# schreibfaul1/ESP32-Opus-Player

Hardware: AMD Instinct MI355X
Metric: decoded 48 kHz stereo frames/sec/GPU (x real-time); HBM GB/s vs roofline (higher is better)
Workload: dtype int32 fixed-point (int16/int32 with 64-bit products); 1 GPU; celt_fb_stereo_64k; streams_per_gpu=65536

## Files before the change

### esp32-opus-player_amd/csrc/og_api.hip

```cpp
#include <hip/hip_runtime.h>
#include <stdio.h>
#include <stdlib.h>
#include <string.h>
#include <condition_variable>
#include <functional>
#include <memory>
#include <new>
#include <mutex>
#include <thread>
#include <vector>
#include "og_decode.hpp"
#include "og_host_framing.hpp"
#include "og_output.hpp"
#include "og_debug.hpp"

using namespace og;

static_assert(sizeof(opusgpu_frame_desc) == sizeof(FrameDesc), "descriptor layout");

#define OG_STALL_MAX_SPINS (1 << 20)
__global__ void __launch_bounds__(64) k_stream_stall(long long ticks, int max_spins) {
    const long long t0 = wall_clock64();
    for (int i = 0; i < max_spins && wall_clock64() - t0 < ticks; i++) __builtin_amdgcn_s_sleep(8);
}
// ... 148 lines not shown
        for (int k = 0; k < max_chunks; k++) consume(k, wa);
    }
    if (p < n) status[p] = st < 0 ? st : (i32)(crc == want);
}

static_assert(sizeof(opusgpu_output_cfg) == sizeof(OutputCfg) && sizeof(OutputCfg) == 4, "output cfg layout");
__global__ void __launch_bounds__(256) k_output_stage(const i16 *__restrict__ pcm, long long pcm_stride, const i32 *__restrict__ valid_of,
                                                       int valid_all, int block_samples, const OutputCfg *__restrict__ cfg_of,
                                                       OutputCfg cfg_all, u32 *__restrict__ out, long long out_stride,
                                                       int units_per_block, long long n_units, int vec_ok) {
    const long long t = (long long)blockIdx.x * 256 + threadIdx.x;
    if (t >= n_units) return;
    const int b = (int)(t / units_per_block), w0 = 4 * (int)(t - (long long)b * units_per_block);
    const OutputCfg c = cfg_of ? cfg_of[b] : cfg_all;
    int valid = valid_of ? valid_of[b] : valid_all;
    valid = valid > block_samples ? block_samples : valid;
    const int count = output_words(c, valid);
    if (w0 >= count) return;
    const i16 *blk = pcm + (size_t)b * pcm_stride;
    u32 *dst = out + (size_t)b * out_stride + w0;
    if (vec_ok && c.bits == 16 && c.channels == 2 && w0 + 4 <= count) {
        const uint4 v = *reinterpret_cast<const uint4 *>(blk + 2 * w0);
        const u32 in[4] = {v.x, v.y, v.z, v.w};
        u32 o[4];
#pragma unroll
        for (int j = 0; j < 4; j++) {
            i32 l = (i32)(i16)(in[j] & 0xffffu), r = (i32)(i16)(in[j] >> 16);
            if (c.force_mono) l = r = (i32)(i16)((l + r) / 2);
            o[j] = output_pack(l, r, false, (i32)c.volume);
        }
        *reinterpret_cast<uint4 *>(dst) = make_uint4(o[0], o[1], o[2], o[3]);
    } else {
        for (int j = 0; j < 4 && w0 + j < count; j++) dst[j] = output_word(blk, w0 + j, c);
    }
}

#ifndef OG_WAVES_PER_SIMD
#define OG_WAVES_PER_SIMD 1
#endif
#define OG_RECON_WAVES 2
#define OG_SILK_WAVES 2
__global__ void __launch_bounds__(64, OG_WAVES_PER_SIMD) k_decode_step(const FrameDesc *__restrict__ descs, const u8 *__restrict__ arena,
                                                   StreamState *st, i16 *pcm, i32 *result, int n, int n_streams,
                                                   int pcm_stride, int skip_celt, SilkHandoff *handoff, const SilkRec *srecs,
                                                   int q4_only) {
    unsigned long long todo = 1ull;
    int base = (int)blockIdx.x;
    if (q4_only) {
        base = (int)blockIdx.x * 64;
        const int f0 = base + (int)threadIdx.x;
        bool mine = false;
        if (f0 < n) {
            const FrameDesc d0 = descs[f0];
            mine = d0.stream >= 0 && d0.stream < n_streams && !desc_rfc(d0.flags) && desc_mode(d0.flags) == MODE_SILK && handoff[f0].valid == 2;
        }
        todo = __ballot(mine);
    }
    while (todo) {
        const int f = base + (int)__builtin_ctzll(todo);
        todo &= todo - 1;
        if (f >= n) return;
        const FrameDesc d = descs[f];
        int ret;
        if (d.stream < 0 || d.stream >= n_streams) {
            ret = BAD_ARG;
        } else if (desc_rfc(d.flags)) {
            continue;
        } else if (skip_celt && desc_mode(d.flags) == MODE_CELT) {
            continue;
        } else {
            StreamState *s = &st[d.stream];
#ifdef OG_PROF_SINGLE
            OG_PROF_INIT();
#endif
            ret = decode_frame_wave<true>(s, arena + d.offset, d.len, desc_mode(d.flags), desc_bandwidth(d.flags),
                                          desc_channels(d.flags), pcm + (size_t)f * pcm_stride, handoff ? &handoff[f] : nullptr,
                                          srecs ? &srecs[f] : nullptr, q4_only, desc_mode_after(d.flags));
#ifdef OG_PROF_SINGLE
            OG_PROF_FLUSH();
#endif
            if (ret == CONTINUE_SPLIT) continue;
        }
        if (threadIdx.x == 0) result[f] = ret;
        __syncthreads();
    }
}

extern "C" void og_launch_silk_synth(hipStream_t s, const void *descs, const void *arena, void *streams, void *pcm, void *result, int n,
                                     int n_streams, int pcm_stride, void *handoff, const void *srecs, int nb_elsewhere);
extern "C" void og_launch_silk_synth_nb(hipStream_t s, const void *descs, const void *arena, void *streams, void *pcm, void *result, int n,
                                        int n_streams, int pcm_stride, void *handoff, const void *srecs, int nb_elsewhere);

#define OG_SPARSE_WAVES 4
template <int LANES>
OG_DEV void silk_parse_kernel_body(const FrameDesc *__restrict__ descs, const u8 *__restrict__ arena, const StreamState *st, SilkRec *srecs,
                                   SilkHandoff *handoff, int n, int n_streams, SilkShadow *shadow, u32 epoch) {
    silk_tables_load();
    if ((int)threadIdx.x >= LANES) return;
    const int f = (int)blockIdx.x * LANES + (int)threadIdx.x;
    if (f >= n) return;
    const FrameDesc d = descs[f];
    const int mode = desc_mode(d.flags);
    if (d.stream < 0 || d.stream >= n_streams || mode == MODE_CELT || desc_rfc(d.flags)) return;
#ifdef OG_PROF_SPARSE
    OG_PROF_INIT();
#endif
    SilkShadow *const sh = shadow ? &shadow[d.stream] : nullptr;
    const SilkPast past(&st[d.stream], sh, epoch);
    silk_parse_lane(past, arena + d.offset, d.len, mode, desc_bandwidth(d.flags), desc_channels(d.flags), &srecs[f], &handoff[f], sh, epoch,
                    desc_mode_after(d.flags));
#ifdef OG_PROF_SPARSE
    OG_PROF_FLUSH();
#endif
}
__global__ void __launch_bounds__(64, OG_SPARSE_WAVES) k_silk_parse(const FrameDesc *__restrict__ descs, const u8 *__restrict__ arena,
                                                      const StreamState *st, SilkRec *srecs, SilkHandoff *handoff, int n,
                                                      int n_streams, SilkShadow *shadow, u32 epoch) {
    silk_parse_kernel_body<32>(descs, arena, st, srecs, handoff, n, n_streams, shadow, epoch);
}
__global__ void __launch_bounds__(64, OG_SPARSE_WAVES) k_silk_parse64(const FrameDesc *__restrict__ descs, const u8 *__restrict__ arena,
                                                        const StreamState *st, SilkRec *srecs, SilkHandoff *handoff, int n,
                                                        int n_streams, SilkShadow *shadow, u32 epoch) {
    silk_parse_kernel_body<64>(descs, arena, st, srecs, handoff, n, n_streams, shadow, epoch);
}

#define OG_SPARAMS_WAVES 4
__global__ void __launch_bounds__(64, OG_SPARAMS_WAVES) k_silk_params(const FrameDesc *__restrict__ descs, const StreamState *st, SilkRec *srecs,
                                                                       int n, int n_streams, SilkShadow *shadow, u32 epoch) {
    constexpr int FR = OG_PAR_LANES / 2;
    const int ch = (int)threadIdx.x / FR, f = (int)blockIdx.x * FR + (int)threadIdx.x % FR;
    bool act = f < n;
    FrameDesc d = {0, 0, 0, 0};
    if (act) {
        d = descs[f];
        act = !(d.stream < 0 || d.stream >= n_streams || desc_mode(d.flags) == MODE_CELT || desc_rfc(d.flags));
    }
    SilkShadow *const sh = act && shadow ? &shadow[d.stream] : nullptr;
    const SilkParPast past(act ? &st[d.stream] : st, sh, epoch);
    const int mode = desc_mode(d.flags), channels = desc_channels(d.flags);
    SilkParTask t;
    t.skip = 1;
    if (act) silk_params_channel(past, mode, desc_bandwidth(d.flags), channels, &srecs[f], ch, t);
    OG_FULL_SYNC();
    if (act) silk_params_shadow(past, t, channels, &srecs[f], ch, sh, epoch);
}

#define OG_PARSE_KERNEL_NAME k_celt_parse
#include "og_parse_kernel.hpp"
extern "C" void og_launch_celt_parse64(hipStream_t s, int grid, const void *descs, const void *arena, void *streams, void *recs, int n,
                                       int n_streams, const void *handoff, int which, int groups, unsigned *started);
extern "C" int og_celt_parse64_frames(void);

extern "C" void og_launch_celt_recon_fb(hipStream_t s, const void *descs, void *streams, const void *recs, void *rout, int n,
                                        int n_streams, int hybrid, unsigned *started);
extern "C" int og_celt_recon_fb_signals(int n);
extern "C" void og_launch_decode_rfc(hipStream_t s, const void *descs, const void *arena, void *streams, void *pcm, void *result, int n,
                                     int n_streams, int pcm_stride);
__global__ void __launch_bounds__(64, OG_RECON_WAVES) k_celt_recon(const FrameDesc *__restrict__ descs, StreamState *st,
                                                                      const ParseRec *recs, ReconOut *rout, int n,
                                                                      int n_streams, int hybrid, int rest_only) {
    unsigned long long todo = 1ull;
    int base = (int)blockIdx.x;
    if (rest_only) {
        base = (int)blockIdx.x * 64;
        const int f0 = base + (int)threadIdx.x;
        bool mine = false;
        if (f0 < n) {
            const FrameDesc d0 = descs[f0];
            const int m0 = desc_mode(d0.flags);
            if (d0.stream >= 0 && d0.stream < n_streams && (m0 == MODE_CELT || (m0 == MODE_HYBRID && hybrid)) && !desc_rfc(d0.flags)) {
                const u32 fl = recs[f0].flags;
                const bool fast = !(fl & (RF_SKIP | RF_BAD_CELT)) && ((fl >> RF_LM_SHIFT) & 3) == 3 && recs[f0].n_words < REC_MAX_WORDS &&
                                  recs[f0].n_leaves <= FAST_MAX_LEAVES;
                mine = !fast && !(m0 == MODE_HYBRID && (fl & RF_SKIP));
            }
        }
        todo = __ballot(mine);
    }
    while (todo) {
        const int f = base + (int)__builtin_ctzll(todo);
        todo &= todo - 1;
        if (f >= n) return;
        const FrameDesc d = descs[f];
        const int mode = desc_mode(d.flags);
        if (d.stream < 0 || d.stream >= n_streams || !(mode == MODE_CELT || (mode == MODE_HYBRID && hybrid)) || desc_rfc(d.flags)) continue;
        if (mode == MODE_HYBRID && (recs[f].flags & RF_SKIP)) continue;
#if !defined(OG_PROF_PARSE) && !defined(OG_PROF_SINGLE) && !defined(OG_PROF_SPARSE) && !defined(OG_PROF_SSYNTH)
        OG_PROF_INIT();
#endif
        const int pos = OG_UNI(st[d.stream].celt.ring_pos);
        const int ret = celt_recon_wave(&st[d.stream], &recs[f], mode, desc_channels(d.flags), rest_only ? RECON_REST_ONLY : RECON_ALL, desc_mode_after(d.flags));
        if (ret != RECON_NOT_MINE && threadIdx.x == 0) rout[f] = ReconOut{ret, pos};
#if !defined(OG_PROF_PARSE) && !defined(OG_PROF_SINGLE) && !defined(OG_PROF_SPARSE) && !defined(OG_PROF_SSYNTH)
        OG_PROF_FLUSH();
#endif
        __syncthreads();
    }
}

static __device__ __forceinline__ i32 pk_add_sat_i16(i32 a, i32 b) {
    typedef short s2 __attribute__((ext_vector_type(2)));
    const s2 r = __builtin_elementwise_add_sat(__builtin_bit_cast(s2, a), __builtin_bit_cast(s2, b));
    return __builtin_bit_cast(i32, r);
}
__global__ void __launch_bounds__(64) k_celt_post(const FrameDesc *__restrict__ descs, StreamState *st, const ParseRec *recs,
                                                  const ReconOut *__restrict__ rout, i32 *__restrict__ result, i16 *pcm, int n,
                                                  int n_streams, int channels, int pcm_stride, const SilkHandoff *handoff,
                                                  int modes, int others_ran) {
    struct RowInfo {
        const i32 *ring;
        i16 *pcm;
        const i16 *silk;
        int pos, silk_n;
    };
    constexpr int CS = 32, PCS = CS / 4, RSTEP = 64 / PCS;
    __shared__ RowInfo rows[64];
    __shared__ __attribute__((aligned(16))) i32 tin[64][CS + 4];
    __shared__ __attribute__((aligned(16))) i16 tout[64][CS + 8];
    const int lane = (int)threadIdx.x;
    const int t = (int)blockIdx.x * 64 + lane;
    const int f = channels == 2 ? t >> 1 : t, c = channels == 2 ? t & 1 : 0;
    bool live = false, emit = false;
    StreamState *ss = nullptr;
    const i16 *silk = nullptr;
    int silk_n = 0;
    int pos = 0;
    if (f < n) {
        const FrameDesc d = descs[f];
        const int mode = desc_mode(d.flags);
        const bool stream_ok = d.stream >= 0 && d.stream < n_streams;
        if (!(modes >> (d.flags & 3) & 1) || (!stream_ok && !others_ran)) {
            if (c == 0) result[f] = BAD_ARG;
        } else if (stream_ok && (mode == MODE_CELT || (mode == MODE_HYBRID && handoff)) && !desc_rfc(d.flags)) {
            const u32 rf = recs[f].flags;
            if (!(mode == MODE_HYBRID && (rf & RF_SKIP))) {
                const ReconOut ro = rout[f];
                if (c == 0) result[f] = ro.ret;
                if (!(rf & (RF_SKIP | RF_BAD_CELT))) {
                    live = true;
                    ss = &st[d.stream];
                    emit = ro.ret >= 0;
                    pos = ro.pos & RING_MASK;
                    if (mode == MODE_HYBRID) {
                        silk = handoff[f].pcm;
                        silk_n = 960 * desc_channels(d.flags);
                    }
                }
            }
        }
    }
    i16 *out = pcm + (size_t)(f < n ? f : 0) * pcm_stride;
    const bool fast = channels == 2 && __all(live && emit && (pos & (CS - 1)) == 0);
    if (!fast) {
        if (live) celt_post_lane(&ss->celt, c, channels, 960, pos, emit ? out : nullptr, silk, silk_n);
        return;
    }
    rows[lane].ring = ss->celt.ring[c];
    rows[lane].pcm = out;
    rows[lane].silk = silk;
    rows[lane].pos = pos;
    rows[lane].silk_n = silk_n;
    __syncthreads();
    const int q = lane % PCS, r0 = lane / PCS;
    const i32 *src[PCS];
    int spos[PCS];
#pragma unroll
    for (int k = 0; k < PCS; k++) {
        src[k] = rows[r0 + RSTEP * k].ring;
        spos[k] = rows[r0 + RSTEP * k].pos + 4 * q;
    }
    og_v4i v[PCS];
#pragma unroll
    for (int k = 0; k < PCS; k++) v[k] = *reinterpret_cast<const og_v4i *>(src[k] + (spos[k] & RING_MASK));
    i32 m = ss->celt.deemph[c];
    for (int ch = 0; ch < 960 / CS; ch++) {
#pragma unroll
        for (int k = 0; k < PCS; k++) *reinterpret_cast<og_v4i *>(&tin[r0 + RSTEP * k][4 * q]) = v[k];
        if (ch + 1 < 960 / CS) {
#pragma unroll
            for (int k = 0; k < PCS; k++) v[k] = *reinterpret_cast<const og_v4i *>(src[k] + ((spos[k] + CS * (ch + 1)) & RING_MASK));
        }
        __syncthreads();
#pragma unroll
        for (int g8 = 0; g8 < CS / 8; g8++) {
            i16 o[8];
#pragma unroll
            for (int h = 0; h < 2; h++) {
                const og_v4i sv = *reinterpret_cast<const og_v4i *>(&tin[lane][8 * g8 + 4 * h]);
                i32 tt = sv.x + m;
                m = mul16x32_q15(27853, tt);
                o[4 * h + 0] = (i16)sat16(pshr32(tt, 12));
                tt = sv.y + m;
                m = mul16x32_q15(27853, tt);
                o[4 * h + 1] = (i16)sat16(pshr32(tt, 12));
                tt = sv.z + m;
                m = mul16x32_q15(27853, tt);
                o[4 * h + 2] = (i16)sat16(pshr32(tt, 12));
                tt = sv.w + m;
                m = mul16x32_q15(27853, tt);
                o[4 * h + 3] = (i16)sat16(pshr32(tt, 12));
            }
            og_v4i w;
            w.x = (i32)((u32)(u16)o[0] | (u32)(u16)o[1] << 16);
            w.y = (i32)((u32)(u16)o[2] | (u32)(u16)o[3] << 16);
            w.z = (i32)((u32)(u16)o[4] | (u32)(u16)o[5] << 16);
            w.w = (i32)((u32)(u16)o[6] | (u32)(u16)o[7] << 16);
            *reinterpret_cast<og_v4i *>(&tout[lane][8 * g8]) = w;
        }
        __syncthreads();
#pragma unroll
        for (int k = 0; k < PCS / 2; k++) {
            const int fr = r0 + RSTEP * k;
            const og_v2u L = *reinterpret_cast<const og_v2u *>(&tout[2 * fr][4 * q]);
            const og_v2u R = *reinterpret_cast<const og_v2u *>(&tout[2 * fr + 1][4 * q]);
            og_v4i w;
            w.x = (i32)((L.x & 0xffffu) | R.x << 16);
            w.y = (i32)(L.x >> 16 | (R.x & 0xffff0000u));
            w.z = (i32)((L.y & 0xffffu) | R.y << 16);
            w.w = (i32)(L.y >> 16 | (R.y & 0xffff0000u));
            const int at = (CS * ch + 4 * q) * 2;
            const i16 *const sk = rows[2 * fr].silk;
            if (sk && at < rows[2 * fr].silk_n) {
                const og_v4i a = *reinterpret_cast<const og_v4i *>(sk + at);
                w.x = pk_add_sat_i16(w.x, a.x);
                w.y = pk_add_sat_i16(w.y, a.y);
                w.z = pk_add_sat_i16(w.z, a.z);
                w.w = pk_add_sat_i16(w.w, a.w);
            }
            *reinterpret_cast<og_v4i *>(rows[2 * fr].pcm + at) = w;
        }
    }
    ss->celt.deemph[c] = m;
}

#include "og_step.hpp"

const size_t og_parse_rec_bytes = sizeof(ParseRec), og_recon_out_bytes = sizeof(ReconOut), og_silk_handoff_bytes = sizeof(SilkHandoff),
             og_silk_rec_bytes = sizeof(SilkRec);
namespace {
struct StepRange {
    const FrameDesc *dd;
    i16 *pp;
    i32 *rr;
    ParseRec *recs;
    ReconOut *rout;
    SilkHandoff *hh;
    SilkRec *srecs;
    StepRange(const Step &st, size_t f0)
        : dd((const FrameDesc *)st.descs + f0), pp((i16 *)st.pcm + f0 * (size_t)st.pcm_stride), rr((i32 *)st.result + f0),
          recs((ParseRec *)st.recs + f0), rout((ReconOut *)st.rout + f0), hh(st.handoff ? (SilkHandoff *)st.handoff + f0 : nullptr),
          srecs(st.srecs ? (SilkRec *)st.srecs + f0 : nullptr) {}
};
}
void launch_stream_stall(opusgpu_ctx *ctx, hipStream_t q) {
    hipLaunchKernelGGL(k_stream_stall, dim3(1), dim3(64), 0, q, ctx->stall_ticks, (int)OG_STALL_MAX_SPINS);
}
void launch_decode_rfc(opusgpu_ctx *ctx, hipStream_t q, const Step &st) {
    og_launch_decode_rfc(q, st.descs, st.arena, ctx->d_streams, st.pcm, st.result, st.n, ctx->n_streams, st.pcm_stride);
}
void launch_decode_step(opusgpu_ctx *ctx, hipStream_t q, const Step &st, size_t f0, int cnt, int pass) {
    const StepRange r(st, f0);
    hipLaunchKernelGGL(k_decode_step, dim3(pass == 2 ? (cnt + 63) / 64 : cnt), dim3(64), 0, q, r.dd, (const u8 *)st.arena, ctx->d_streams, r.pp,
                       r.rr, cnt, ctx->n_streams, st.pcm_stride, pass ? 1 : 0, pass == 2 ? r.hh : nullptr,
                       (const SilkRec *)(pass == 2 ? r.srecs : nullptr), pass == 2 ? 1 : 0);
}
void launch_silk_parse(opusgpu_ctx *ctx, hipStream_t q, const Step &st, size_t f0, int cnt, void *shadow, uint32_t epoch) {
    const StepRange r(st, f0);
    hipLaunchKernelGGL(k_silk_parse, dim3((cnt + 31) / 32), dim3(64), 0, q, r.dd, (const u8 *)st.arena, (const StreamState *)ctx->d_streams,
                       r.srecs, r.hh, cnt, ctx->n_streams, (SilkShadow *)shadow, epoch);
}
void launch_silk_parse64(opusgpu_ctx *ctx, hipStream_t q, const Step &st, size_t f0, int cnt, void *shadow, uint32_t epoch) {
    const StepRange r(st, f0);
    hipLaunchKernelGGL(k_silk_parse64, dim3((cnt + 63) / 64), dim3(64), 0, q, r.dd, (const u8 *)st.arena, (const StreamState *)ctx->d_streams,
                       r.srecs, r.hh, cnt, ctx->n_streams, (SilkShadow *)shadow, epoch);
}
void launch_silk_params(opusgpu_ctx *ctx, hipStream_t q, const Step &st, size_t f0, int cnt, void *shadow, uint32_t epoch) {
    const StepRange r(st, f0);
    hipLaunchKernelGGL(k_silk_params, dim3((cnt + OG_PAR_LANES / 2 - 1) / (OG_PAR_LANES / 2)), dim3(64), 0, q, r.dd,
                       (const StreamState *)ctx->d_streams, r.srecs, cnt, ctx->n_streams, (SilkShadow *)shadow, epoch);
}
int celt_parse_early_grid(const opusgpu_ctx *ctx, int cnt, bool wide) {
    const int per = (wide ? og_celt_parse64_frames() : OG_PL_FRAMES) * ctx->parse_groups;
    return (cnt + per - 1) / per;
}
void launch_celt_parse(opusgpu_ctx *ctx, hipStream_t q, const Step &st, size_t f0, int cnt, bool wide, bool early) {
    const StepRange r(st, f0);
    const int which = early ? (int)PARSE_CELT_ONLY : (int)PARSE_ALL, groups = early ? ctx->parse_groups : 1;
    const int per = wide ? og_celt_parse64_frames() : OG_PL_FRAMES;
    const int grid = early ? celt_parse_early_grid(ctx, cnt, wide) : (cnt + per - 1) / per;
    u32 *const started = early ? ctx->sp.d_started : nullptr;
    if (wide)
        og_launch_celt_parse64(q, grid, r.dd, st.arena, ctx->d_streams, r.recs, cnt, ctx->n_streams, r.hh, which, groups, started);
    else
        hipLaunchKernelGGL(k_celt_parse, dim3(grid), dim3(64 * OG_PL_WAVES), 0, q, r.dd, (const u8 *)st.arena, ctx->d_streams, r.recs, cnt,
                           ctx->n_streams, (const SilkHandoff *)r.hh, which, groups, started);
}
void launch_celt_recon_fb(opusgpu_ctx *ctx, hipStream_t q, const Step &st, size_t f0, int cnt, bool counts_in) {
    const StepRange r(st, f0);
    og_launch_celt_recon_fb(q, r.dd, ctx->d_streams, r.recs, r.rout, cnt, ctx->n_streams, r.hh ? 1 : 0, counts_in ? ctx->sp.d_started + 16 : nullptr);
}
void launch_celt_recon(opusgpu_ctx *ctx, hipStream_t q, const Step &st, size_t f0, int cnt) {
    const StepRange r(st, f0);
    hipLaunchKernelGGL(k_celt_recon, dim3(ctx->fast_recon ? (cnt + 63) / 64 : cnt), dim3(64), 0, q, r.dd, ctx->d_streams, (const ParseRec *)r.recs,
                       r.rout, cnt, ctx->n_streams, r.hh ? 1 : 0, ctx->fast_recon);
}
void launch_celt_post(opusgpu_ctx *ctx, hipStream_t q, const Step &st, size_t f0, int cnt, bool others) {
    const StepRange r(st, f0);
    hipLaunchKernelGGL(k_celt_post, dim3((cnt * ctx->channels + 63) / 64), dim3(64), 0, q, r.dd, ctx->d_streams, (const ParseRec *)r.recs,
                       (const ReconOut *)r.rout, r.rr, r.pp, cnt, ctx->n_streams, ctx->channels, st.pcm_stride, (const SilkHandoff *)r.hh, st.modes,
                       others ? 1 : 0);
}
void launch_silk_synth(opusgpu_ctx *ctx, hipStream_t q, const Step &st, size_t f0, int cnt, int nb_done) {
    const StepRange r(st, f0);
    og_launch_silk_synth(q, r.dd, st.arena, ctx->d_streams, r.pp, r.rr, cnt, ctx->n_streams, st.pcm_stride, r.hh, r.srecs, nb_done);
}
void launch_silk_synth_nb(opusgpu_ctx *ctx, hipStream_t q, const Step &st, size_t f0, int cnt) {
    const StepRange r(st, f0);
    og_launch_silk_synth_nb(q, r.dd, st.arena, ctx->d_streams, r.pp, r.rr, cnt, ctx->n_streams, st.pcm_stride, r.hh, r.srecs, 1);
}


extern "C" {


int opusgpu_version(void) { return 100; }

int opusgpu_ctx_create(int device, opusgpu_ctx **out) {
    if (!out || device < 0) return OPUSGPU_BAD_ARG;
    *out = nullptr;
    int count = 0;
    if (hipGetDeviceCount(&count) != hipSuccess || count <= 0 || device >= count) return OPUSGPU_ERR_NO_DEVICE;
    if (hipSetDevice(device) != hipSuccess) return OPUSGPU_ERR_NO_DEVICE;
    hipFuncAttributes attr;
    if (hipFuncGetAttributes(&attr, reinterpret_cast<const void *>(k_decode_step)) != hipSuccess) {
        (void)hipGetLastError();
        return OPUSGPU_ERR_NO_DEVICE;
    }
    opusgpu_ctx *ctx = new (std::nothrow) opusgpu_ctx();
    if (!ctx) return OPUSGPU_ALLOC_FAIL;
    ctx->device = device;
    ctx->split_celt = og_debug().split;
    ctx->split_hybrid = og_debug().split_hybrid;
    ctx->fast_recon = og_debug().fast_recon;
    ctx->parse_groups = og_debug().parse_groups;
    ctx->host_parts = og_debug().host_parts;
    if (og_debug().stall_us) {
        int khz = 0;
        if (hipDeviceGetAttribute(&khz, hipDeviceAttributeWallClockRate, device) != hipSuccess || khz <= 0) {
            (void)hipGetLastError();
            delete ctx;
            return OPUSGPU_ERR_HIP;
        }
        ctx->stall_ticks = (long long)og_debug().stall_us * khz / 1000;
    }
    if (hipStreamCreateWithFlags(&ctx->stream, hipStreamNonBlocking) != hipSuccess) {
        delete ctx;
        return OPUSGPU_ERR_HIP;
    }
    *out = ctx;
    return OPUSGPU_OK;
}

void opusgpu_ctx_destroy(opusgpu_ctx *ctx) {
    if (!ctx) return;
    (void)hipSetDevice(ctx->device);
    (void)hipStreamSynchronize(ctx->stream);
    (void)hipFree(ctx->d_streams);
    (void)hipFree(ctx->d_descs);
    (void)hipFree(ctx->d_arena);
    (void)hipFree(ctx->d_pcm);
    (void)hipFree(ctx->d_result);
    pipeline_destroy(ctx);
    for (int i = 0; i < 6; i++) {
        (void)hipFree(ctx->d_recs[i]);
        (void)hipFree(ctx->d_rout[i]);
    }
    for (int i = 0; i < OG_SILK_SETS; i++) {
        (void)hipFree(ctx->d_handoff[i]);
        (void)hipFree(ctx->d_srecs[i]);
    }
    (void)hipFree(ctx->d_shadow);
    (void)hipHostFree(ctx->h_pcm);
    (void)hipHostFree(ctx->h_res);
    (void)hipHostFree(ctx->h_arena);
    (void)hipHostFree(ctx->h_descs);
    (void)hipFree(ctx->d_crc_tables);
    for (hipEvent_t e : ctx->ev_piece)
        if (e) (void)hipEventDestroy(e);
    for (hipEvent_t e : ctx->ev_part)
        if (e) (void)hipEventDestroy(e);
    if (ctx->copy_stream) (void)hipStreamDestroy(ctx->copy_stream);
    (void)hipStreamDestroy(ctx->stream);
    delete ctx;
}

const char *opusgpu_last_error(const opusgpu_ctx *ctx) { return ctx ? ctx->err : "no context"; }
int opusgpu_set_mode(opusgpu_ctx *ctx, int mode) {
    if (!ctx || (mode != OPUSGPU_MODE_REFERENCE && mode != OPUSGPU_MODE_RFC)) return OPUSGPU_BAD_ARG;
    ctx->mode = mode;
    return OPUSGPU_OK;
}
int opusgpu_get_mode(const opusgpu_ctx *ctx) { return ctx ? ctx->mode : OPUSGPU_MODE_REFERENCE; }
int opusgpu_set_pipeline(opusgpu_ctx *ctx, int on) {
    if (!ctx) return OPUSGPU_BAD_ARG;
    HIPCHK(ctx, hipSetDevice(ctx->device));
    if (on)
        if (int rc = pipeline_create(ctx)) return rc;
    if ((on != 0) != (ctx->pipeline != 0)) {
        HIPCHK(ctx, hipDeviceSynchronize());
        ctx->sp.drained();
        ctx->sp.last_kind = 0;
        ctx->sp.shadow_epoch++;
    }
    ctx->pipeline = on ? 1 : 0;
    return OPUSGPU_OK;
}
int opusgpu_get_pipeline(const opusgpu_ctx *ctx) { return ctx ? ctx->pipeline : 0; }
size_t opusgpu_stream_state_bytes(void) { return sizeof(StreamState); }
int opusgpu_stream_count(const opusgpu_ctx *ctx) { return ctx ? ctx->n_streams : 0; }
int opusgpu_stream_channels(const opusgpu_ctx *ctx) { return ctx ? ctx->channels : 0; }

int opusgpu_streams_reset(opusgpu_ctx *ctx, int first, int count, int full) {
    if (!ctx || first < 0 || count < 0 || first + count > ctx->n_streams) return OPUSGPU_BAD_ARG;
    if (count == 0) return OPUSGPU_OK;
    HIPCHK(ctx, hipSetDevice(ctx->device));
    if (int rc = sync_in_flight(ctx)) return rc;
    ctx->sp.drained();
    ctx->sp.shadow_epoch++;
    hipLaunchKernelGGL(k_stream_init, dim3(count), dim3(64), 0, ctx->stream, ctx->d_streams, first, count, ctx->channels,
                       full ? 1 : 0);
    HIPCHK(ctx, hipGetLastError());
    HIPCHK(ctx, hipStreamSynchronize(ctx->stream));
    for (int i = first; i < first + count; i++) ctx->last_count[i] = ctx->last_flags[i] = 0;
    return OPUSGPU_OK;
}

int opusgpu_streams_alloc(opusgpu_ctx *ctx, int n_streams, int channels) {
    if (!ctx || n_streams <= 0 || (channels != 1 && channels != 2)) return OPUSGPU_BAD_ARG;
    HIPCHK(ctx, hipSetDevice(ctx->device));
    HIPCHK(ctx, hipStreamSynchronize(ctx->stream));
    if (int rc = sync_in_flight(ctx)) return rc;
    if (ctx->d_streams) {
        HIPCHK(ctx, hipFree(ctx->d_streams));
        ctx->d_streams = nullptr;
        ctx->n_streams = 0;
    }
    hipError_t e = hipMalloc((void **)&ctx->d_streams, sizeof(StreamState) * (size_t)n_streams);
    if (e != hipSuccess) return fail(ctx, OPUSGPU_ALLOC_FAIL, "hipMalloc(streams)", e);
    if (ctx->d_shadow) HIPCHK(ctx, hipFree(ctx->d_shadow));
    ctx->d_shadow = nullptr;
    e = hipMalloc(&ctx->d_shadow, sizeof(SilkShadow) * (size_t)n_streams);
    if (e != hipSuccess) return fail(ctx, OPUSGPU_ALLOC_FAIL, "hipMalloc(shadow)", e);
    HIPCHK(ctx, hipMemset(ctx->d_shadow, 0, sizeof(SilkShadow) * (size_t)n_streams));
    ctx->sp.shadow_epoch++;
// ... 368 lines not shown
```

### esp32-opus-player_amd/csrc/og_ctx.hpp

```cpp
#pragma once
#include <hip/hip_runtime_api.h>
#include <stdint.h>
#include <stdio.h>
#include <condition_variable>
#include <functional>
#include <mutex>
#include <thread>
#include <utility>
#include <vector>
#include "../../include/opusgpu.h"
#include "og_debug.hpp"

namespace og {
struct StreamState;
}
enum { OPUSGPU_COPY_PIECES = 16, OPUSGPU_COPY_THREADS = 8 };

struct HostPool {
    std::vector<std::thread> th;
    std::mutex m;
    std::condition_variable wake, done;
    std::function<void(int)> job;
    int generation = 0, want = 0, pending = 0;
    bool quit = false;
    ~HostPool() {
        {
            std::lock_guard<std::mutex> l(m);
            quit = true;
        }
        wake.notify_all();
        for (auto &t : th) t.join();
    }
    void worker(int id) {
        int seen = 0;
        for (;;) {
            std::function<void(int)> f;
            {
                std::unique_lock<std::mutex> l(m);
                wake.wait(l, [&] { return quit || (generation != seen && id < want); });
                if (quit) return;
                seen = generation;
                f = job;
            }
            f(id);
            {
                std::lock_guard<std::mutex> l(m);
                if (--pending == 0) done.notify_all();
            }
        }
    }
    void run(int count, const std::function<void(int)> &f) {
        if (count <= 1) {
            f(0);
            return;
        }
        while ((int)th.size() < count - 1) {
            const int id = (int)th.size();
            th.emplace_back([this, id] { worker(id); });
        }
        {
            std::lock_guard<std::mutex> l(m);
            job = [&f](int id) { f(id + 1); };
            want = count - 1;
            pending = count - 1;
            generation++;
        }
        wake.notify_all();
        f(0);
        std::unique_lock<std::mutex> l(m);
        done.wait(l, [&] { return pending == 0; });
    }
};

struct LoudnessState {
    opusgpu_loudness_req req{};
    std::vector<opusgpu_loudness> records;
    std::vector<double> gains;
};

struct opusgpu_ctx {
    int device = -1;
    hipStream_t stream = nullptr;
    og::StreamState *d_streams = nullptr;
    int n_streams = 0, channels = 0;
    void *d_descs = nullptr, *d_arena = nullptr, *d_pcm = nullptr, *d_result = nullptr;
    size_t cap_descs = 0, cap_arena = 0, cap_pcm = 0, cap_result = 0;
    void *h_pcm = nullptr, *h_res = nullptr;
    size_t cap_h_pcm = 0, cap_h_res = 0;
    void *h_arena = nullptr, *h_descs = nullptr;
    size_t cap_h_arena = 0, cap_h_descs = 0;
    HostPool pool;
    uint32_t *d_crc_tables = nullptr;
    hipEvent_t ev_piece[OPUSGPU_COPY_PIECES] = {};
    hipStream_t copy_stream = nullptr;
    std::mutex registered_mutex;
    std::vector<std::pair<uintptr_t, size_t>> registered;
    hipEvent_t ev_part[OPUSGPU_COPY_PIECES] = {};
    int host_parts = 8;
    void *d_recs[6] = {}, *d_rout[6] = {};
    size_t cap_recs[6] = {}, cap_rout[6] = {};
    void *d_handoff[OG_SILK_SETS] = {}, *d_srecs[OG_SILK_SETS] = {};
    size_t cap_handoff[OG_SILK_SETS] = {}, cap_srecs[OG_SILK_SETS] = {};
    const void *last_srecs = nullptr;
    void *d_shadow = nullptr;
    StepPipeline sp;
    int split_celt = 1;
    int split_hybrid = 1;
    int fast_recon = 1;
    int mode = OPUSGPU_MODE_REFERENCE;
    int pipeline = 0;
    long long stall_ticks = 0;
    const void *last_recs = nullptr;
    int parse_groups = 1;
    const void *last_descs = nullptr;
    int last_n = 0, last_had_silk_recs = 0;
    std::vector<int32_t> last_count, last_flags;
    LoudnessState loud;
    char err[256] = {0};
};

static int fail(opusgpu_ctx *ctx, int code, const char *what, hipError_t e) {
    if (ctx) snprintf(ctx->err, sizeof(ctx->err), "%s: %s", what, hipGetErrorString(e));
    return code;
}
#define HIPCHK(ctx, call)                                                \
    do {                                                                 \
        hipError_t e_ = (call);                                          \
        if (e_ != hipSuccess) return fail(ctx, OPUSGPU_ERR_HIP, #call, e_); \
    } while (0)
static int grow(opusgpu_ctx *ctx, void **p, size_t *cap, size_t need);
```

### esp32-opus-player_amd/csrc/og_debug.hpp

```cpp
#pragma once
#include <stdlib.h>
#include <string.h>

struct og_debug_knobs {
    int split = 1, split_hybrid = 1, fast_recon = 1, hybrid_recon_aside = 1, silk_params_aside = 1, silk_nb_kernel = 1, halves = 1, silk_pipeline = 1, hybrid_pipeline = 1, parse_wide = 1, parse_groups = 1, parse_priority = 1, host_parts = 16, host_slices = 1, host_timing = 0,
        pages_timing = 0, launch_delay_us = 0, stall_stream = 0, stall_us = 0;
};
inline const og_debug_knobs &og_debug() {
    static const og_debug_knobs k = [] {
        og_debug_knobs v;
        auto flag = [](const char *name, int &field) {
            if (const char *e = getenv(name)) field = e[0] != '0' && e[0] != '\0';
        };
        auto number = [](const char *name, int &field, int lo, int hi) {
            if (const char *e = getenv(name)) {
                const int x = atoi(e);
                if (x >= lo && x <= hi) field = x;
            }
        };
        flag("OPUSGPU_SPLIT", v.split);
        flag("OPUSGPU_SPLIT_HYBRID", v.split_hybrid);
        flag("OPUSGPU_FAST_RECON", v.fast_recon);
        number("OPUSGPU_HYBRID_RECON_ASIDE", v.hybrid_recon_aside, 0, 2);
        flag("OPUSGPU_SILK_PARAMS_ASIDE", v.silk_params_aside);
        flag("OPUSGPU_SILK_NB_KERNEL", v.silk_nb_kernel);
        flag("OPUSGPU_HALVES", v.halves);
        flag("OPUSGPU_SILK_PIPELINE", v.silk_pipeline);
        flag("OPUSGPU_HYBRID_PIPELINE", v.hybrid_pipeline);
        number("OPUSGPU_PARSE_WIDE", v.parse_wide, 0, 2);
        number("OPUSGPU_PARSE_GROUPS", v.parse_groups, 1, 8);
        flag("OPUSGPU_PARSE_PRIORITY", v.parse_priority);
        if (const char *e = getenv("OPUSGPU_HOST_PARTS")) {
            const int x = atoi(e);
            if (x == 1 || x == 2 || x == 4 || x == 8 || x == 16) v.host_parts = x;
        }
        flag("OPUSGPU_HOST_SLICES", v.host_slices);
        if (const char *e = getenv("OPUSGPU_HOST_TIMING")) v.host_timing = atoi(e) == 2 ? 2 : 1;
        v.pages_timing = getenv("OPUSGPU_PAGES_TIMING") != nullptr;
        number("OPUSGPU_LAUNCH_DELAY_US", v.launch_delay_us, 0, 100000);
        if (const char *e = getenv("OPUSGPU_STALL_STREAM")) {
            const char *names[] = {"step", "parse", "recon", "side"};
            for (int i = 0; i < 4; i++)
                if (!strcmp(e, names[i])) v.stall_stream = i + 1;
        }
        if (const char *e = getenv("OPUSGPU_STALL_US")) {
            const int x = atoi(e);
            v.stall_us = x < 0 ? 0 : x > 100000 ? 100000 : x;
        }
        if (!v.stall_stream || !v.stall_us) v.stall_stream = v.stall_us = 0;
        return v;
    }();
    return k;
}
```

### esp32-opus-player_amd/csrc/og_recon.hip

```cpp
#define OG_RECON_TIGHT 1
#include <hip/hip_runtime.h>
#include "og_celt_recon.hpp"

using namespace og;

#define OG_FAST_WAVES 6


__global__ void __launch_bounds__(64, OG_FAST_WAVES) k_celt_recon_fb(const FrameDesc *__restrict__ descs, StreamState *st,
                                                                           const ParseRec *recs, ReconOut *rout, int n, int n_streams,
                                                                           int hybrid, u32 *started) {
    if (started && threadIdx.x == 0 && (blockIdx.x & 63) == 0) __hip_atomic_fetch_add(started, 1u, __ATOMIC_RELAXED, __HIP_MEMORY_SCOPE_SYSTEM);
    const int f = (int)blockIdx.x;
    StreamState *sp = nullptr;
    const ParseRec *rec = nullptr;
    ReconCtx rx;
    rx.leaves = false;
    rx.flags = 0;
    bool mine = false;
    int pos = 0;
    u32 lg = 0, la = 0, li = 0;
    OG_PROF_INIT();
    if (f < n) {
        rec = &recs[f];
        const FrameDesc d = descs[f];
        const int lane = OG_LANE;
        const i32 w_rec = reinterpret_cast<const i32 *>(rec)[lane < 16 ? lane : 15];
        {
            typedef u32 u32x4 __attribute__((ext_vector_type(4)));
            const u32x4 lf = *reinterpret_cast<const u32x4 *>(&rec->leaf[lane]);
            li = lf[0];
            lg = lf[1];
            la = lf[2];
        }
        rx.pre_bandE = rec->bandE[lane < 2 * NBANDS ? lane : 0];
        rx.pre_pulses = rec->pulses[lane < NBANDS ? lane : 0];
        rx.pre_band_w = rec->band_w[lane < NBANDS ? lane : 0];
        const int mode = desc_mode(d.flags);
        bool ok = !(d.stream < 0 || d.stream >= n_streams || !(mode == MODE_CELT || (mode == MODE_HYBRID && hybrid)) || desc_rfc(d.flags));
        if (ok) {
            sp = &st[d.stream];
            const i32 w_st = recon_hdr_fetch(sp, rec);
            rx.pre_logE1 = sp->celt.logE1[lane < 2 * NBANDS ? lane : 0];
            rx.pre_logE2 = sp->celt.logE2[lane < 2 * NBANDS ? lane : 0];
            rx.pre = true;
            recon_hdr_unpack(lane < 16 ? w_rec : w_st, rx.h);
            if (mode == MODE_HYBRID && (rx.h.flags & RF_SKIP)) ok = false;
        }
        if (ok) {
            pos = rx.h.ring_pos;
            mine = recon_begin(sp, rec, mode, desc_channels(d.flags), RECON_FAST_ONLY, rx);
            if (mine) {
                if (OG_LANE == 0) rout[f] = ReconOut{recon_result(rx), pos};
                recon_bookkeeping(sp, rx);
                rx.booked = true;
            }
        }
    }
    if (mine && rx.leaves) {
        pvq_tab_load();
        OG_SYNC();
        recon_leaves_own(rec, rx, true, lg, la, li);
    }
    if (mine) recon_finish(sp, rec, rx);
    OG_PROF_FLUSH();
}

extern "C" void og_launch_celt_recon_fb(hipStream_t s, const void *descs, void *streams, const void *recs, void *rout, int n,
                                        int n_streams, int hybrid, unsigned *started) {
    hipLaunchKernelGGL(k_celt_recon_fb, dim3(n), dim3(64), 0, s, (const FrameDesc *)descs, (StreamState *)streams,
                       (const ParseRec *)recs, (ReconOut *)rout, n, n_streams, hybrid, started);
}
extern "C" int og_celt_recon_fb_signals(int n) { return (n + 63) / 64; }

#ifdef OG_PROF
extern "C" int og_recon_fb_prof(unsigned long long *out64, int reset) {
    if (hipMemcpyFromSymbol(out64, HIP_SYMBOL(g_prof), sizeof(unsigned long long) * 64) != hipSuccess) return -1;
    if (reset) {
        unsigned long long z[64] = {0};
        if (hipMemcpyToSymbol(HIP_SYMBOL(g_prof), z, sizeof(z)) != hipSuccess) return -1;
    }
    return 0;
}
#endif
```

Baseline: 50.57 million frames/s.

## Fold empty CELT frames into fb recon and slim post kernel addressing

The fast full-band recon kernel now also handles CELT frames flagged bad-but-not-skipped (the empty or rest case) when a new debug knob is on. The separate rest-only recon launch is then skipped for that step, removing one kernel launch and its pass over the frames. Separately, the post kernel drops its shared-memory row table and the second output buffer. It recomputes ring addresses from the stream index via shuffles and 32-bit offsets, uses wave-uniform pointers for the PCM and SILK rows, and reuses one LDS tile with an extra barrier per chunk. It also sets launch bounds to 5 waves, and the new fast path only applies when the stream state array fits a 32-bit 16-byte index.

```diff
diff --git a/esp32-opus-player_amd/csrc/og_api.hip b/esp32-opus-player_amd/csrc/og_api.hip
--- a/esp32-opus-player_amd/csrc/og_api.hip
+++ b/esp32-opus-player_amd/csrc/og_api.hip
@@ -324,7 +324,7 @@
 extern "C" int og_celt_parse64_frames(void);
 
 extern "C" void og_launch_celt_recon_fb(hipStream_t s, const void *descs, void *streams, const void *recs, void *rout, int n,
-                                        int n_streams, int hybrid, unsigned *started);
+                                        int n_streams, int hybrid, unsigned *started, int empties);
 extern "C" int og_celt_recon_fb_signals(int n);
 extern "C" void og_launch_decode_rfc(hipStream_t s, const void *descs, const void *arena, void *streams, void *pcm, void *result, int n,
                                      int n_streams, int pcm_stride);
@@ -375,20 +375,20 @@
     const s2 r = __builtin_elementwise_add_sat(__builtin_bit_cast(s2, a), __builtin_bit_cast(s2, b));
     return __builtin_bit_cast(i32, r);
 }
-__global__ void __launch_bounds__(64) k_celt_post(const FrameDesc *__restrict__ descs, StreamState *st, const ParseRec *recs,
+template <class T>
+static __device__ __forceinline__ T *uniform_ptr(T *p) {
+    const unsigned long long a = (unsigned long long)p;
+    return (T *)((unsigned long long)(u32)__builtin_amdgcn_readfirstlane((int)(u32)a) |
+                 (unsigned long long)(u32)__builtin_amdgcn_readfirstlane((int)(u32)(a >> 32)) << 32);
+}
+#define OG_POST_WAVES 5
+__global__ void __launch_bounds__(64, OG_POST_WAVES) k_celt_post(const FrameDesc *__restrict__ descs, StreamState *st, const ParseRec *recs,
                                                   const ReconOut *__restrict__ rout, i32 *__restrict__ result, i16 *pcm, int n,
                                                   int n_streams, int channels, int pcm_stride, const SilkHandoff *handoff,
                                                   int modes, int others_ran) {
-    struct RowInfo {
-        const i32 *ring;
-        i16 *pcm;
-        const i16 *silk;
-        int pos, silk_n;
-    };
     constexpr int CS = 32, PCS = CS / 4, RSTEP = 64 / PCS;
-    __shared__ RowInfo rows[64];
+    static_assert(RSTEP % 2 == 0, "a lane's rows are all of one channel");
     __shared__ __attribute__((aligned(16))) i32 tin[64][CS + 4];
-    __shared__ __attribute__((aligned(16))) i16 tout[64][CS + 8];
     const int lane = (int)threadIdx.x;
     const int t = (int)blockIdx.x * 64 + lane;
     const int f = channels == 2 ? t >> 1 : t, c = channels == 2 ? t & 1 : 0;
@@ -396,9 +396,10 @@
     StreamState *ss = nullptr;
     const i16 *silk = nullptr;
     int silk_n = 0;
-    int pos = 0;
+    int pos = 0, stream = 0;
     if (f < n) {
         const FrameDesc d = descs[f];
+        stream = d.stream;
         const int mode = desc_mode(d.flags);
         const bool stream_ok = d.stream >= 0 && d.stream < n_streams;
         if (!(modes >> (d.flags & 3) & 1) || (!stream_ok && !others_ran)) {
@@ -422,35 +423,40 @@
         }
     }
     i16 *out = pcm + (size_t)(f < n ? f : 0) * pcm_stride;
-    const bool fast = channels == 2 && __all(live && emit && (pos & (CS - 1)) == 0);
+    const bool fast = channels == 2 && (size_t)n_streams * sizeof(StreamState) <= (size_t)16 << 32 && __all(live && emit && (pos & (CS - 1)) == 0);
     if (!fast) {
         if (live) celt_post_lane(&ss->celt, c, channels, 960, pos, emit ? out : nullptr, silk, silk_n);
         return;
     }
-    rows[lane].ring = ss->celt.ring[c];
-    rows[lane].pcm = out;
-    rows[lane].silk = silk;
-    rows[lane].pos = pos;
-    rows[lane].silk_n = silk_n;
-    __syncthreads();
     const int q = lane % PCS, r0 = lane / PCS;
-    const i32 *src[PCS];
-    int spos[PCS];
+    constexpr u32 STATE16 = sizeof(StreamState) / 16, RING16 = (offsetof(StreamState, celt) + offsetof(CeltState, ring)) / 16, CHAN16 = RING * 4 / 16;
+    static_assert(sizeof(StreamState) % 16 == 0 && (offsetof(StreamState, celt) + offsetof(CeltState, ring)) % 16 == 0 && RING / CS <= 256, "ring pieces");
+    u32 row16[PCS], at_chunk[PCS / 4] = {};
 #pragma unroll
     for (int k = 0; k < PCS; k++) {
-        src[k] = rows[r0 + RSTEP * k].ring;
-        spos[k] = rows[r0 + RSTEP * k].pos + 4 * q;
-    }
+        row16[k] = (u32)__shfl(stream, r0 + RSTEP * k) * STATE16 + RING16 + (u32)(r0 & 1) * CHAN16 + (u32)q;
+        at_chunk[k / 4] |= (u32)(__shfl(pos, r0 + RSTEP * k) / CS) << (8 * (k % 4));
+    }
+    auto piece = [&](int k, int chunk) -> og_v4i {
+        const u32 at = ((at_chunk[k / 4] >> (8 * (k % 4)) & 255u) + (u32)chunk) & (u32)(RING / CS - 1);
+        return *reinterpret_cast<const og_v4i *>(reinterpret_cast<const char *>(st) + (size_t)(row16[k] + at * (CS * 4 / 16)) * 16);
+    };
+    const size_t f_wave = (size_t)blockIdx.x * 32;
+    const u32 lane_pcm = 2u * (u32)(r0 * pcm_stride + 8 * q), lane_sk = (u32)r0 * (u32)sizeof(SilkHandoff) + 16u * (u32)q;
+    u32 sk_960 = 0;
+#pragma unroll
+    for (int k = 0; k < PCS / 2; k++) sk_960 |= (u32)(__shfl(silk_n, 2 * (r0 + RSTEP * k)) / 960) << (8 * k);
     og_v4i v[PCS];
 #pragma unroll
-    for (int k = 0; k < PCS; k++) v[k] = *reinterpret_cast<const og_v4i *>(src[k] + (spos[k] & RING_MASK));
-    i32 m = ss->celt.deemph[c];
+    for (int k = 0; k < PCS; k++) v[k] = piece(k, 0);
+    i32 m = st[stream].celt.deemph[c];
     for (int ch = 0; ch < 960 / CS; ch++) {
+        if (ch) __syncthreads();
 #pragma unroll
         for (int k = 0; k < PCS; k++) *reinterpret_cast<og_v4i *>(&tin[r0 + RSTEP * k][4 * q]) = v[k];
         if (ch + 1 < 960 / CS) {
 #pragma unroll
-            for (int k = 0; k < PCS; k++) v[k] = *reinterpret_cast<const og_v4i *>(src[k] + ((spos[k] + CS * (ch + 1)) & RING_MASK));
+            for (int k = 0; k < PCS; k++) v[k] = piece(k, ch + 1);
         }
         __syncthreads();
 #pragma unroll
@@ -477,32 +483,33 @@
             w.y = (i32)((u32)(u16)o[2] | (u32)(u16)o[3] << 16);
             w.z = (i32)((u32)(u16)o[4] | (u32)(u16)o[5] << 16);
             w.w = (i32)((u32)(u16)o[6] | (u32)(u16)o[7] << 16);
-            *reinterpret_cast<og_v4i *>(&tout[lane][8 * g8]) = w;
+            *reinterpret_cast<og_v4i *>(&tin[lane][4 * g8]) = w;
         }
         __syncthreads();
 #pragma unroll
         for (int k = 0; k < PCS / 2; k++) {
             const int fr = r0 + RSTEP * k;
-            const og_v2u L = *reinterpret_cast<const og_v2u *>(&tout[2 * fr][4 * q]);
-            const og_v2u R = *reinterpret_cast<const og_v2u *>(&tout[2 * fr + 1][4 * q]);
+            const og_v2u L = *reinterpret_cast<const og_v2u *>(&tin[2 * fr][2 * q]);
+            const og_v2u R = *reinterpret_cast<const og_v2u *>(&tin[2 * fr + 1][2 * q]);
             og_v4i w;
             w.x = (i32)((L.x & 0xffffu) | R.x << 16);
             w.y = (i32)(L.x >> 16 | (R.x & 0xffff0000u));
             w.z = (i32)((L.y & 0xffffu) | R.y << 16);
             w.w = (i32)(L.y >> 16 | (R.y & 0xffff0000u));
             const int at = (CS * ch + 4 * q) * 2;
-            const i16 *const sk = rows[2 * fr].silk;
-            if (sk && at < rows[2 * fr].silk_n) {
-                const og_v4i a = *reinterpret_cast<const og_v4i *>(sk + at);
+            if (at < 960 * (int)(sk_960 >> (8 * k) & 255u)) {
+                const char *const sk = uniform_ptr(reinterpret_cast<const char *>(handoff[f_wave + RSTEP * k].pcm + 2 * CS * ch));
+                const og_v4i a = *reinterpret_cast<const og_v4i *>(sk + lane_sk);
                 w.x = pk_add_sat_i16(w.x, a.x);
                 w.y = pk_add_sat_i16(w.y, a.y);
                 w.z = pk_add_sat_i16(w.z, a.z);
                 w.w = pk_add_sat_i16(w.w, a.w);
             }
-            *reinterpret_cast<og_v4i *>(rows[2 * fr].pcm + at) = w;
-        }
-    }
-    ss->celt.deemph[c] = m;
+            char *const to = uniform_ptr(reinterpret_cast<char *>(pcm + (f_wave + RSTEP * k) * pcm_stride + 2 * CS * ch));
+            *reinterpret_cast<og_v4i *>(to + lane_pcm) = w;
+        }
+    }
+    st[stream].celt.deemph[c] = m;
 }
 
 #include "og_step.hpp"
@@ -569,9 +576,15 @@
 }
 void launch_celt_recon_fb(opusgpu_ctx *ctx, hipStream_t q, const Step &st, size_t f0, int cnt, bool counts_in) {
     const StepRange r(st, f0);
-    og_launch_celt_recon_fb(q, r.dd, ctx->d_streams, r.recs, r.rout, cnt, ctx->n_streams, r.hh ? 1 : 0, counts_in ? ctx->sp.d_started + 16 : nullptr);
+    ctx->recon_fb_took_rest = counts_in && !r.hh && st.modes == 4 && og_debug().rest_in_fb;
+    og_launch_celt_recon_fb(q, r.dd, ctx->d_streams, r.recs, r.rout, cnt, ctx->n_streams, r.hh ? 1 : 0, counts_in ? ctx->sp.d_started + 16 : nullptr,
+                            ctx->recon_fb_took_rest ? 1 : 0);
 }
 void launch_celt_recon(opusgpu_ctx *ctx, hipStream_t q, const Step &st, size_t f0, int cnt) {
+    if (ctx->fast_recon && ctx->recon_fb_took_rest) {
+        ctx->recon_fb_took_rest = false;
+        return;
+    }
     const StepRange r(st, f0);
     hipLaunchKernelGGL(k_celt_recon, dim3(ctx->fast_recon ? (cnt + 63) / 64 : cnt), dim3(64), 0, q, r.dd, ctx->d_streams, (const ParseRec *)r.recs,
                        r.rout, cnt, ctx->n_streams, r.hh ? 1 : 0, ctx->fast_recon);
diff --git a/esp32-opus-player_amd/csrc/og_ctx.hpp b/esp32-opus-player_amd/csrc/og_ctx.hpp
--- a/esp32-opus-player_amd/csrc/og_ctx.hpp
+++ b/esp32-opus-player_amd/csrc/og_ctx.hpp
@@ -107,6 +107,7 @@
     int split_celt = 1;
     int split_hybrid = 1;
     int fast_recon = 1;
+    bool recon_fb_took_rest = false;
     int mode = OPUSGPU_MODE_REFERENCE;
     int pipeline = 0;
     long long stall_ticks = 0;
diff --git a/esp32-opus-player_amd/csrc/og_debug.hpp b/esp32-opus-player_amd/csrc/og_debug.hpp
--- a/esp32-opus-player_amd/csrc/og_debug.hpp
+++ b/esp32-opus-player_amd/csrc/og_debug.hpp
@@ -3,7 +3,7 @@
 #include <string.h>
 
 struct og_debug_knobs {
-    int split = 1, split_hybrid = 1, fast_recon = 1, hybrid_recon_aside = 1, silk_params_aside = 1, silk_nb_kernel = 1, halves = 1, silk_pipeline = 1, hybrid_pipeline = 1, parse_wide = 1, parse_groups = 1, parse_priority = 1, host_parts = 16, host_slices = 1, host_timing = 0,
+    int split = 1, split_hybrid = 1, fast_recon = 1, rest_in_fb = 1, hybrid_recon_aside = 1, silk_params_aside = 1, silk_nb_kernel = 1, halves = 1, silk_pipeline = 1, hybrid_pipeline = 1, parse_wide = 1, parse_groups = 1, parse_priority = 1, host_parts = 16, host_slices = 1, host_timing = 0,
         pages_timing = 0, launch_delay_us = 0, stall_stream = 0, stall_us = 0;
 };
 inline const og_debug_knobs &og_debug() {
@@ -21,6 +21,7 @@
         flag("OPUSGPU_SPLIT", v.split);
         flag("OPUSGPU_SPLIT_HYBRID", v.split_hybrid);
         flag("OPUSGPU_FAST_RECON", v.fast_recon);
+        flag("OPUSGPU_REST_IN_FB", v.rest_in_fb);
         number("OPUSGPU_HYBRID_RECON_ASIDE", v.hybrid_recon_aside, 0, 2);
         flag("OPUSGPU_SILK_PARAMS_ASIDE", v.silk_params_aside);
         flag("OPUSGPU_SILK_NB_KERNEL", v.silk_nb_kernel);
diff --git a/esp32-opus-player_amd/csrc/og_recon.hip b/esp32-opus-player_amd/csrc/og_recon.hip
--- a/esp32-opus-player_amd/csrc/og_recon.hip
+++ b/esp32-opus-player_amd/csrc/og_recon.hip
@@ -9,7 +9,7 @@
 
 __global__ void __launch_bounds__(64, OG_FAST_WAVES) k_celt_recon_fb(const FrameDesc *__restrict__ descs, StreamState *st,
                                                                            const ParseRec *recs, ReconOut *rout, int n, int n_streams,
-                                                                           int hybrid, u32 *started) {
+                                                                           int hybrid, u32 *started, int empties) {
     if (started && threadIdx.x == 0 && (blockIdx.x & 63) == 0) __hip_atomic_fetch_add(started, 1u, __ATOMIC_RELAXED, __HIP_MEMORY_SCOPE_SYSTEM);
     const int f = (int)blockIdx.x;
     StreamState *sp = nullptr;
@@ -49,7 +49,8 @@
         }
         if (ok) {
             pos = rx.h.ring_pos;
-            mine = recon_begin(sp, rec, mode, desc_channels(d.flags), RECON_FAST_ONLY, rx);
+            const int role = empties && mode == MODE_CELT && (rx.h.flags & (RF_SKIP | RF_BAD_CELT)) == RF_BAD_CELT ? (int)RECON_REST_ONLY : (int)RECON_FAST_ONLY;
+            mine = recon_begin(sp, rec, mode, desc_channels(d.flags), role, rx);
             if (mine) {
                 if (OG_LANE == 0) rout[f] = ReconOut{recon_result(rx), pos};
                 recon_bookkeeping(sp, rx);
@@ -67,9 +68,9 @@
 }
 
 extern "C" void og_launch_celt_recon_fb(hipStream_t s, const void *descs, void *streams, const void *recs, void *rout, int n,
-                                        int n_streams, int hybrid, unsigned *started) {
+                                        int n_streams, int hybrid, unsigned *started, int empties) {
     hipLaunchKernelGGL(k_celt_recon_fb, dim3(n), dim3(64), 0, s, (const FrameDesc *)descs, (StreamState *)streams,
-                       (const ParseRec *)recs, (ReconOut *)rout, n, n_streams, hybrid, started);
+                       (const ParseRec *)recs, (ReconOut *)rout, n, n_streams, hybrid, started, empties);
 }
 extern "C" int og_celt_recon_fb_signals(int n) { return (n + 63) / 64; }
 
```

Result: faster. 52.44 million frames/s (median of 6 runs) (+3.7%).
